# paninski-lab/eks

Hardware: AMD Instinct MI355X
Metric: frames*keypoints smoothed/s + achieved HBM GB/s fraction, singlecam 100k x 256 (higher is better)
Workload: dtype f32

## Files before the change

eks_amd/csrc/eks_diag.hip:

```cpp
#include <hip/hip_runtime.h>

#include <cstdlib>

#include "eks_diag_lane.hpp"
#include "eks_internal.hpp"
#include "eks_win_walk.hpp"

namespace eks {

struct LaneMap {
  int N, T, nc;
  int nt_log2;
  int ntile;
  int reverse;
};

__device__ __forceinline__ bool lane_coords(const LaneMap& L, int& n, int& j) {
  const int wave = blockIdx.x * (blockDim.x >> 6) + (threadIdx.x >> 6);
  const int lane = threadIdx.x & 63;
  const int tile = wave % L.ntile;
  const int cg = wave / L.ntile;
  const int nt = 1 << L.nt_log2;
  n = tile * nt + (lane & (nt - 1));
  j = cg * (64 >> L.nt_log2) + (lane >> L.nt_log2);
// ... 404 lines not shown
}

template <int B, bool UNIT, int VS_ROW>
__device__ __forceinline__ void replay_window_block(const BlockMap& L, const DiagModel& M, const WinWs& Wn,
                                                    const float* __restrict__ y, const float* __restrict__ var,
                                                    float* __restrict__ ms, float* __restrict__ Vs) {
  __shared__ float sh[5][kWinW][64];
  __shared__ float shy[64];
  const int w = __builtin_amdgcn_readfirstlane(threadIdx.x >> 6), lane = threadIdx.x & 63;
  const int tile = L.tile0 + blockIdx.x % L.ntile;
  int wg = blockIdx.x / L.ntile;
  if (L.reverse) wg = Wn.nwg - 1 - wg;
  const int n = tile * 64 + lane;
  constexpr int VW = VS_ROW == 0 ? 1 : VS_ROW;
  const bool slow = n >= L.N || (Wn.slow != nullptr && Wn.slow[n] != 0);
  if (__ballot(!slow) == 0) return;
  const int jh0 = wg * kWinG - kWinH;
  const int j = jh0 + w;
  const bool valid = j >= 0 && j < L.nc;
  const bool live = n < L.N && valid;
  ChainParams<float> p{1.f, 1.f, 0.f};
  const int t0 = valid ? j * B : 0;
  const int len = valid ? min(B, L.T - t0) : 0;
  const bool full = len == B;
  const size_t first = (size_t)t0 * L.N + (size_t)tile * 64;
  const BufferRows rows{rows_rsrc(y + first), rows_rsrc(var + first), (unsigned)lane * 4, (unsigned)L.N * 4};
  float v0[B], v1[B];
  Elem<float> own = elem_identity<float>();
  float y0 = 0.f;
  if (live) {
    p = load_chain_params(M, n);
    if (full) {
      load_rows<B, true>(rows, B, v0, v1);
      y0 = v0[0];
      own = summarize_loaded<B, UNIT, true>(v0, v1, B, p);
    } else {
      load_rows<B, false>(rows, len, v0, v1);
      y0 = v0[0];
      own = summarize_loaded<B, UNIT, false>(v0, v1, len, p);
    }
  }
  sh[0][w][lane] = own.A; sh[1][w][lane] = own.b; sh[2][w][lane] = own.C; sh[3][w][lane] = own.eta;
  sh[4][w][lane] = own.J;
  if (w == 0) shy[lane] = y0;
  __syncthreads();
  const int wo = w - kWinH;
  if (wo < 0 || wo >= kWinG || !live) return;
  auto lds_elem = [&](int q) {
    return Elem<float>{sh[0][q][lane], sh[1][q][lane], sh[2][q][lane], sh[3][q][lane], sh[4][q][lane]};
  };
  const bool cut_front = jh0 <= 0, cut_back = (wg + 1) * kWinG + kWinH >= L.nc;
  Elem<float> hf = lds_elem(0), hb = lds_elem(kWinH + kWinG);
#pragma unroll
  for (int q = 1; q < kWinH; ++q) {
    hf = elem_combine(hf, lds_elem(q));
    hb = elem_combine(hb, lds_elem(kWinH + kWinG + q));
  }
  float m, P;
  load_chain_prior(M, n, m, P);
  if (!cut_front) m = UNIT ? shy[lane] : shy[lane] * rcp(p.c);
  const bool good = !slow && fabsf(m) <= 3e38f && (cut_front || fabsf(hf.A) <= kWinTol) &&
                    (cut_back || fabsf(hb.A) <= kWinTol);
  if (!good && !slow && wo == 0 && Wn.fail != nullptr) {
    Wn.fail[(size_t)wg * L.N + n] = 1;
    atomicOr(&Wn.gate[tile], 1);
  }
  elem_apply(hf, m, P);
  for (int q = 0; q < wo; ++q) elem_apply(lds_elem(kWinH + q), m, P);
  if (full) filter_loaded<B, UNIT, true>(v0, v1, B, p, m, P);
  else filter_loaded<B, UNIT, false>(v0, v1, len, p, m, P);
  float eta = 0.f, J = 0.f;
  elem_back(hb, eta, J);
  for (int q = kWinG - 1; q > wo; --q) elem_back(lds_elem(kWinH + q), eta, J);
  fuse_info(m, P, eta, J);
  if (Wn.nan_bad && !good) m = P = __builtin_nanf("");
  const BufferStore<VS_ROW> st{rows_rsrc(ms + first), rows_rsrc(Vs + first * VW), (unsigned)lane * 4,
                               (unsigned)L.N * 4, n % M.D};
  if (good || Wn.nan_bad) {
    if (full) smooth_rows<B, UNIT, true>(v0, v1, B, p, m, P, st);
    else smooth_rows<B, UNIT, false>(v0, v1, len, p, m, P, st);
  }
}

template <int B, bool UNIT, int VS_ROW>
__device__ __forceinline__ void replay_walk_block(const BlockMap& L, const DiagModel& M, const WinWs& Wn,
                                                  const float* __restrict__ y, const float* __restrict__ var,
                                                  float* __restrict__ ms, float* __restrict__ Vs) {
  __shared__ float sh[5][kWalkRing][64];
  __shared__ float shy[kWalkStand][64];
  const int w = __builtin_amdgcn_readfirstlane(threadIdx.x >> 6), lane = threadIdx.x & 63;
  const int tile = L.tile0 + blockIdx.x % L.ntile;
  const int run_len = Wn.run_len;
  int run = blockIdx.x / L.ntile;
  if (L.reverse) run = (Wn.nwg + run_len - 1) / run_len - 1 - run;
  const int n = tile * 64 + lane;
  constexpr int VW = VS_ROW == 0 ? 1 : VS_ROW;
  const bool slow = n >= L.N || (Wn.slow != nullptr && Wn.slow[n] != 0);
  if (__ballot(!slow) == 0) return;
  ChainParams<float> p{1.f, 1.f, 0.f};
  float m0 = 0.f, P0 = 0.f;
  if (n < L.N) {
    p = load_chain_params(M, n);
    load_chain_prior(M, n, m0, P0);
  }
  const int d = n % M.D;
  float v0[B], v1[B];
  const int g0 = run * run_len, g1 = min(g0 + run_len, Wn.nwg);
  for (int g = g0; g < g1; ++g) {
    const int base = walk_base(g);
    const int off = walk_off(g, w);
    const int j = base + off;
    const bool valid = j >= 0 && j < L.nc;
    const bool live = n < L.N && valid;
    const int t0 = valid ? j * B : 0;
    const int len = valid ? min(B, L.T - t0) : 0;
    const bool full = len == B;
    const size_t first = (size_t)t0 * L.N + (size_t)tile * 64;
    if (walk_loads(off, g == g0)) {
      Elem<float> own = elem_identity<float>();
      float y0 = 0.f;
      if (live) {
        const BufferRows rows{rows_rsrc(y + first), rows_rsrc(var + first), (unsigned)lane * 4, (unsigned)L.N * 4};
        if (full) {
          load_rows<B, true>(rows, B, v0, v1);
          y0 = v0[0];
          own = summarize_loaded<B, UNIT, true>(v0, v1, B, p);
        } else {
          load_rows<B, false>(rows, len, v0, v1);
          y0 = v0[0];
          own = summarize_loaded<B, UNIT, false>(v0, v1, len, p);
        }
      }
      const int slot = walk_elem_slot(j);
      sh[0][slot][lane] = own.A; sh[1][slot][lane] = own.b; sh[2][slot][lane] = own.C; sh[3][slot][lane] = own.eta;
      sh[4][slot][lane] = own.J;
      if (walk_saves_stand(j)) shy[walk_stand_slot(j)][lane] = y0;
    }
    __syncthreads();
    if (!walk_replays(off) || !live) continue;
    const int wo = off - kWinH;
    auto lds_elem = [&](int jj) {
      const int q = walk_elem_slot(jj);
      return Elem<float>{sh[0][q][lane], sh[1][q][lane], sh[2][q][lane], sh[3][q][lane], sh[4][q][lane]};
    };
    const bool cut_front = base <= 0, cut_back = (g + 1) * kWinG + kWinH >= L.nc;
    Elem<float> hf = lds_elem(base), hb = lds_elem(base + kWinH + kWinG);
#pragma unroll
    for (int q = 1; q < kWinH; ++q) {
      hf = elem_combine(hf, lds_elem(base + q));
      hb = elem_combine(hb, lds_elem(base + kWinH + kWinG + q));
    }
    float m = m0, P = P0;
    if (!cut_front) {
      const float ys = shy[walk_stand_slot(base)][lane];
      m = UNIT ? ys : ys * rcp(p.c);
    }
    const bool good = !slow && fabsf(m) <= 3e38f && (cut_front || fabsf(hf.A) <= kWinTol) &&
                      (cut_back || fabsf(hb.A) <= kWinTol);
    if (!good && !slow && wo == 0 && Wn.fail != nullptr) {
      Wn.fail[(size_t)g * L.N + n] = 1;
      atomicOr(&Wn.gate[tile], 1);
    }
    elem_apply(hf, m, P);
    for (int q = 0; q < wo; ++q) elem_apply(lds_elem(base + kWinH + q), m, P);
    if (full) filter_loaded<B, UNIT, true>(v0, v1, B, p, m, P);
    else filter_loaded<B, UNIT, false>(v0, v1, len, p, m, P);
    float eta = 0.f, J = 0.f;
    elem_back(hb, eta, J);
    for (int q = kWinG - 1; q > wo; --q) elem_back(lds_elem(base + kWinH + q), eta, J);
    fuse_info(m, P, eta, J);
    if (Wn.nan_bad && !good) m = P = __builtin_nanf("");
    const BufferStore<VS_ROW> st{rows_rsrc(ms + first), rows_rsrc(Vs + first * VW), (unsigned)lane * 4,
                                 (unsigned)L.N * 4, d};
    if (good || Wn.nan_bad) {
      if (full) smooth_rows<B, UNIT, true>(v0, v1, B, p, m, P, st);
      else smooth_rows<B, UNIT, false>(v0, v1, len, p, m, P, st);
    }
  }
}

constexpr int kFormElems = 0;
constexpr int kFormRecompute = 1;
constexpr int kFormWindow = 2;
constexpr int kFormWalk = 3;

template <int B, bool UNIT, int VS_ROW, int FORM>
__global__ __launch_bounds__(FORM >= kFormWindow ? 64 * kWinW : 64 * kFW) void diag_replay_blk_kernel(
    BlockMap L, DiagModel M, DiagWs W, ScanWs S, WinWs Wn, const float* __restrict__ y, const float* __restrict__ var,
    float* __restrict__ ms, float* __restrict__ Vs) {
  if constexpr (FORM == kFormWalk) {
    replay_walk_block<B, UNIT, VS_ROW>(L, M, Wn, y, var, ms, Vs);
  } else if constexpr (FORM == kFormWindow) {
    replay_window_block<B, UNIT, VS_ROW>(L, M, Wn, y, var, ms, Vs);
  } else if constexpr (FORM == kFormRecompute) {
    replay_recompute_block<B, UNIT, VS_ROW, false>(L, M, S, Wn, y, var, ms, Vs);
  } else {
    const int w = __builtin_amdgcn_readfirstlane(threadIdx.x >> 6), lane = threadIdx.x & 63;
    const int tile = L.tile0 + blockIdx.x % L.ntile;
    int grp = blockIdx.x / L.ntile;
    if (L.reverse) grp = L.ngrp - 1 - grp;
    const int n = tile * 64 + lane, j = grp * kFW + w;
    const int j0 = grp * kFW, j1 = min(j0 + kFW, L.nc);
    constexpr int VW = VS_ROW == 0 ? 1 : VS_ROW;
    if (n >= L.N || j >= L.nc) return;
    const ChainParams<float> p = load_chain_params(M, n);
    const int t0 = j * B;
    const int len = min(B, L.T - t0);
    const bool full = len == B;
    const size_t first = (size_t)t0 * L.N + (size_t)tile * 64;
    const BufferRows rows{rows_rsrc(y + first), rows_rsrc(var + first), (unsigned)lane * 4, (unsigned)L.N * 4};
    float v0[B], v1[B];
    if (full) load_rows<B, true>(rows, B, v0, v1);
    else load_rows<B, false>(rows, len, v0, v1);
    Elem<float> ef[kFW - 1];
#pragma unroll
    for (int q = 0; q < kFW - 1; ++q)
      if (j0 + q < j) ef[q] = load_elem(W, (size_t)(j0 + q) * L.N + n);
    const size_t ob = (size_t)grp * L.N + n;
    float m = S.bm[ob], P = S.bP[ob], eta = S.bEta[ob], J = S.bJ[ob];
#pragma unroll
    for (int q = 0; q < kFW - 1; ++q)
      if (j0 + q < j) elem_apply(ef[q], m, P);
    Elem<float> eb[kFW - 1];
#pragma unroll
    for (int q = 0; q < kFW - 1; ++q)
      if (j + 1 + q < j1) eb[q] = load_elem(W, (size_t)(j + 1 + q) * L.N + n);
    if (full) filter_loaded<B, UNIT, true>(v0, v1, B, p, m, P);
    else filter_loaded<B, UNIT, false>(v0, v1, len, p, m, P);
#pragma unroll
    for (int q = kFW - 2; q >= 0; --q)
      if (j + 1 + q < j1) elem_back(eb[q], eta, J);
    fuse_info(m, P, eta, J);
    const BufferStore<VS_ROW> st{rows_rsrc(ms + first), rows_rsrc(Vs + first * VW), (unsigned)lane * 4,
                                 (unsigned)L.N * 4, n % M.D};
    if (full) smooth_rows<B, UNIT, true>(v0, v1, B, p, m, P, st);
    else smooth_rows<B, UNIT, false>(v0, v1, len, p, m, P, st);
  }
}

template <int B, bool UNIT, int VS_ROW>
__global__ __launch_bounds__(64 * kFW) void diag_replay_exact_kernel(BlockMap L, DiagModel M, ScanWs S, WinWs Wn,
                                                                    const float* __restrict__ y,
                                                                    const float* __restrict__ var,
                                                                    float* __restrict__ ms,
                                                                    float* __restrict__ Vs) {
  replay_recompute_block<B, UNIT, VS_ROW, true>(L, M, S, Wn, y, var, ms, Vs);
}

__global__ __launch_bounds__(64 * kProbeWin) void diag_window_probe_kernel(int N, int T, DiagModel M, WinWs Wn,
                                                                          const float* __restrict__ var,
                                                                          int classify) {
  __shared__ int bad[kProbeWin][64];
  const int w = __builtin_amdgcn_readfirstlane(threadIdx.x >> 6), lane = threadIdx.x & 63;
  const int tile = blockIdx.x, n = tile * 64 + lane;
  for (int i = threadIdx.x; i < Wn.nwg * 64; i += 64 * kProbeWin) {
    const int c = tile * 64 + (i & 63);
    if (c < N) Wn.fail[(size_t)(i >> 6) * N + c] = 0;
  }
  int s = 0;
  if (classify && n < N) {
    const ChainParams<float> p = load_chain_params(M, n);
    const int t0 = (int)((long long)w * (T - kProbeLen) / (kProbeWin - 1));
    const float* v = var + (size_t)t0 * N + n;
    float r[kProbeLen];
#pragma unroll
    for (int i = 0; i < kProbeLen; ++i) r[i] = v[(size_t)i * N];
    float A = 1.f, C = 0.f;
#pragma unroll
    for (int i = 0; i < kProbeLen; ++i) {
      const float ri = clip_var(r[i]);
      const float rg = ri * rcp(ri + C * p.c * p.c);
      A = p.times_a(A * rg);
      C = p.times_a2(C * rg) + p.q_s;
    }
// ... 78 lines not shown
#pragma unroll
    for (int i = 0; i < PER; ++i)
      if (b0 + i < q1) {
        const size_t o = (size_t)(b0 + i) * N + n;
        S.bm[o] = m;
        S.bP[o] = P;
        elem_apply(e[i], m, P);
      }
  }
  for (int b1 = q1; b1 > q0; b1 -= PER) {
    const int lo = max(q0, b1 - PER);
    if (!held) {
#pragma unroll
      for (int i = 0; i < PER; ++i)
        if (lo + i < b1) e[i] = agg(lo + i);
    }
#pragma unroll
    for (int i = PER - 1; i >= 0; --i)
      if (lo + i < b1) {
        const size_t o = (size_t)(lo + i) * N + n;
        S.bEta[o] = eta;
        S.bJ[o] = J;
        elem_back(e[i], eta, J);
      }
  }
}

#ifndef EKS_DIAG_CHUNK
#define EKS_DIAG_CHUNK 32
#endif
constexpr int kChunk = EKS_DIAG_CHUNK;

static inline size_t plane_bytes(int nc, int N) { return align_up((size_t)nc * N * sizeof(float), 256); }

static inline size_t win_slow_bytes(int N) { return align_up((size_t)N, 256); }
static inline size_t win_fail_bytes(int nc, int N) { return align_up((size_t)((nc + kWinG - 1) / kWinG) * N, 256); }
static inline size_t win_bytes(int nc, int N) {
  return win_slow_bytes(N) + win_fail_bytes(nc, N) + align_up((size_t)((N + 63) / 64) * sizeof(int), 256);
}

size_t diag_smooth_workspace_bytes(int T, int N) {
  const int nc = (T + kChunk - 1) / kChunk;
  const int nblk = (nc + kFW - 1) / kFW;
  return 9 * plane_bytes(nc, N) + 9 * plane_bytes(nblk, N) + win_bytes(nc, N);
}

static LaneMap make_lane_map(int T, int N, int B) {
  LaneMap L;
  L.N = N;
  L.T = T;
  L.nc = (T + B - 1) / B;
  int nt_log2 = 0;
  while ((1 << nt_log2) < N && nt_log2 < 6) ++nt_log2;
  L.nt_log2 = nt_log2;
  L.ntile = (N + (1 << nt_log2) - 1) >> nt_log2;
  L.reverse = 0;
  return L;
}

template <bool UNIT>
static void launch_replay(int vs_row, dim3 grid, hipStream_t st, const LaneMap& L, const DiagModel& M,
                          const DiagWs& W, const float* y, const float* var, float* ms, float* Vs) {
#define EKS_REPLAY(R)                                                                             \
  case R:                                                                                         \
    hipLaunchKernelGGL((diag_replay_kernel<kChunk, UNIT, R>), grid, dim3(256), 0, st, L, M, W, y, \
                       var, ms, Vs);                                                              \
    break;
  switch (vs_row) {
    EKS_REPLAY(0)
    EKS_REPLAY(1)
    EKS_REPLAY(2)
    EKS_REPLAY(3)
    EKS_REPLAY(4)
    EKS_REPLAY(5)
    EKS_REPLAY(6)
    EKS_REPLAY(7)
    EKS_REPLAY(8)
  }
#undef EKS_REPLAY
}

constexpr int kWalkDefault = 1;
constexpr int kWalkMinRun = 2;

static int device_cu_count() {
  static const int n = [] {
    int dev = 0, c = 0;
    if (hipGetDevice(&dev) != hipSuccess ||
        hipDeviceGetAttribute(&c, hipDeviceAttributeMultiprocessorCount, dev) != hipSuccess || c <= 0)
      c = 256;
    return c;
  }();
  return n;
}

static int walk_run(int ntile, int nwg) {
  if (knob_int(KNOB_SMOOTH_WINDOW_WALK, kWalkDefault) == 0) return 0;
  if (knob_set(KNOB_SMOOTH_WINDOW_RUN)) return min(max(knob_int(KNOB_SMOOTH_WINDOW_RUN, 1), 1), nwg);
  thread_local int c_ntile = 0, c_nwg = 0, c_run = 0;
  if (ntile != c_ntile || nwg != c_nwg) {
    c_run = walk_run_length(ntile, nwg, device_cu_count());
    c_ntile = ntile;
    c_nwg = nwg;
  }
  return c_run >= kWalkMinRun ? c_run : 0;
}

int diag_smooth(const eks_dims_t& d, const float* y, const float* var, const DiagModel& M,
                float* ms, float* Vs, void* ws, size_t ws_bytes, hipStream_t st) {
  const int T = d.n_frames, D = d.state_dim, N = d.n_keypoints * D;
  const bool vs_diag = d.flags & EKS_FLAG_VS_DIAG;
  if (!vs_diag && D > 8) return EKS_ERR_UNSUPPORTED;
  if (ws_bytes < diag_smooth_workspace_bytes(T, N)) return EKS_ERR_WORKSPACE;
  const LaneMap Lf = make_lane_map(T, N, kChunk);
  const LaneMap& L = Lf;
  const size_t pb = plane_bytes(L.nc, N);
  char* base = static_cast<char*>(ws);
  DiagWs W;
  float** planes[9] = {&W.eA, &W.eb, &W.eC, &W.eEta, &W.eJ, &W.pm, &W.pP, &W.sEta, &W.sJ};
  for (int i = 0; i < 9; ++i) *planes[i] = reinterpret_cast<float*>(base + i * pb);
  const int ngrp_f = (L.nc + kFW - 1) / kFW;
  const bool in_range = (size_t)kChunk * N * (vs_diag ? 1 : D) * sizeof(float) < ((size_t)1 << 31);
  const bool fused = L.nt_log2 == 6 && in_range &&
                     (knob_set(KNOB_SMOOTH_UNFUSED) ? knob_int(KNOB_SMOOTH_UNFUSED, 0) == 0 : ngrp_f <= 1024);
  ScanWs S;
  S.nblk = fused ? (L.nc + kFW - 1) / kFW : (L.nc + kScanCB - 1) / kScanCB;
  const size_t sb = plane_bytes(S.nblk, N);
  float** splanes[9] = {&S.gA, &S.gb, &S.gC, &S.gEta, &S.gJ, &S.bm, &S.bP, &S.bEta, &S.bJ};
  for (int i = 0; i < 9; ++i) *splanes[i] = reinterpret_cast<float*>(base + 9 * pb + i * sb);
  const int vs_row = vs_diag ? 0 : D;
  const bool unit = d.flags & EKS_FLAG_UNIT_AC;
  const int k1_reverse = knob_int(KNOB_SUMMARIZE_REVERSE, 0) == 1 ? 1 : 0;
  const int k3_reverse = knob_set(KNOB_REPLAY_FORWARD) ? (knob_int(KNOB_REPLAY_FORWARD, 0) == 1 ? 0 : 1) : !k1_reverse;
  const int win_mode = knob_int(KNOB_SMOOTH_WINDOW, kWinDefault);
  const int win_min_t = max(kProbeLen, knob_int(KNOB_SMOOTH_WINDOW_MIN_T, kWinMinT));
  const bool windowed = fused && win_mode != 0 && T >= win_min_t;
  WinWs Wn{nullptr, nullptr, nullptr, (L.nc + kWinG - 1) / kWinG, 0, 0};
  if (windowed) {
    char* wb = base + 9 * pb + 9 * sb;
    if (win_mode == 2) {
      Wn.nan_bad = 1;
    } else {
      Wn.slow = reinterpret_cast<unsigned char*>(wb);
      Wn.fail = reinterpret_cast<unsigned char*>(wb + win_slow_bytes(N));
      Wn.gate = reinterpret_cast<int*>(wb + win_slow_bytes(N) + win_fail_bytes(L.nc, N));
    }
  }
  const int* gate = windowed ? Wn.gate : nullptr;
  if (fused) {
    const bool rc_all = knob_set(KNOB_REPLAY_RECOMPUTE) ? knob_int(KNOB_REPLAY_RECOMPUTE, 0) == 1
                                                        : 5 * pb >= ((size_t)16 << 20);
    const int tp = L.ntile;
    for (int tile0 = 0; tile0 < L.ntile; tile0 += tp) {
    const int ntl = min(tp, L.ntile - tile0);
    const int n0 = tile0 * 64, Np = min(N - n0, ntl * 64);
    BlockMap Bm{N, T, L.nc, ntl, S.nblk, k1_reverse, tile0};
    const dim3 bgrid((unsigned)((long)Bm.ntile * Bm.ngrp)), bblock(64 * kFW);
    const bool rc = rc_all || windowed;
#define EKS_K1_BLK(UN)                                                                                  \
  do {                                                                                                  \
    if (rc)                                                                                             \
      hipLaunchKernelGGL((diag_summarize_blk_kernel<kChunk, UN, true>), bgrid, bblock, 0, st, Bm, M, W, \
                         S, y, var, gate);                                                              \
    else                                                                                                \
      hipLaunchKernelGGL((diag_summarize_blk_kernel<kChunk, UN, false>), bgrid, bblock, 0, st, Bm, M,   \
                         W, S, y, var, gate);                                                           \
  } while (0)
#define EKS_K3_BLK(UN, R)                                                                               \
  do {                                                                                                  \
    if (windowed)                                                                                       \
      hipLaunchKernelGGL((diag_replay_exact_kernel<kChunk, UN, R>), bgrid, bblock, 0, st, Bm, M, S, Wn, \
                         y, var, ms, Vs);                                                               \
    else if (rc)                                                                                        \
      hipLaunchKernelGGL((diag_replay_blk_kernel<kChunk, UN, R, kFormRecompute>), bgrid, bblock, 0, st, \
                         Bm, M, W, S, Wn, y, var, ms, Vs);                                              \
    else                                                                                                \
      hipLaunchKernelGGL((diag_replay_blk_kernel<kChunk, UN, R, kFormElems>), bgrid, bblock, 0, st, Bm, \
                         M, W, S, Wn, y, var, ms, Vs);                                                  \
  } while (0)
#define EKS_K3_WIN(UN, R)                                                                               \
  hipLaunchKernelGGL((diag_replay_blk_kernel<kChunk, UN, R, kFormWindow>), wgrid, dim3(64 * kWinW), 0,  \
                     st, Bw, M, W, S, Wn, y, var, ms, Vs)
#define EKS_K3_WALK(UN, R)                                                                             \
  hipLaunchKernelGGL((diag_replay_blk_kernel<kChunk, UN, R, kFormWalk>), wgrid, dim3(64 * kWinW), 0,    \
                     st, Bw, M, W, S, Ww, y, var, ms, Vs)
#define EKS_REPLAY_WIN(R)                                                                              \
  case R:                                                                                              \
    if (run_len > 0) {                                                                                 \
      if (unit)                                                                                        \
        EKS_K3_WALK(true, R);                                                                          \
      else                                                                                             \
        EKS_K3_WALK(false, R);                                                                         \
    } else if (unit)                                                                                   \
      EKS_K3_WIN(true, R);                                                                             \
    else                                                                                               \
      EKS_K3_WIN(false, R);                                                                            \
    break;
    if (windowed) {
      if (win_mode != 2) {
        ProfScope ps("diag_window_probe", st);
        hipLaunchKernelGGL(diag_window_probe_kernel, dim3(ntl), dim3(64 * kProbeWin), 0, st, N, T, M, Wn, var,
                           knob_int(KNOB_SMOOTH_WINDOW_PROBE, 1) != 0 ? 1 : 0);
      }
      {
        ProfScope ps("diag_replay", st);
        BlockMap Bw = Bm;
        Bw.reverse = k3_reverse;
        const int run_len = walk_run(Bw.ntile, Wn.nwg);
        WinWs Ww = Wn;
        Ww.run_len = run_len;
        const dim3 wgrid((unsigned)((long)Bw.ntile * (run_len > 0 ? (Wn.nwg + run_len - 1) / run_len : Wn.nwg)));
        switch (vs_row) {
          EKS_REPLAY_WIN(0)
          EKS_REPLAY_WIN(1)
          EKS_REPLAY_WIN(2)
          EKS_REPLAY_WIN(3)
          EKS_REPLAY_WIN(4)
          EKS_REPLAY_WIN(5)
          EKS_REPLAY_WIN(6)
          EKS_REPLAY_WIN(7)
          EKS_REPLAY_WIN(8)
        }
      }
      if (win_mode == 2) continue;
    }
    {
      ProfScope ps("diag_summarize", st);
      if (unit)
        EKS_K1_BLK(true);
      else
        EKS_K1_BLK(false);
    }
    {
      ProfScope ps("diag_scan", st);
      const bool ch4 = knob_set(KNOB_SCAN_CH) ? knob_int(KNOB_SCAN_CH, 4) == 4 : Np < 2048;
      const bool per8 = (S.nblk + 63) / 64 <= 8;
      const int Ne = n0 + Np;
      if (ch4) {
        if (per8)
          hipLaunchKernelGGL((diag_scan_groups_kernel<8, 4>), dim3((Np + 3) / 4), dim3(256), 0, st, N, n0, Ne, M, S, gate);
        else
          hipLaunchKernelGGL((diag_scan_groups_kernel<16, 4>), dim3((Np + 3) / 4), dim3(256), 0, st, N, n0, Ne, M, S, gate);
      } else {
        if (per8)
          hipLaunchKernelGGL((diag_scan_groups_kernel<8, 16>), dim3((Np + 15) / 16), dim3(1024), 0, st, N, n0, Ne, M, S, gate);
        else
          hipLaunchKernelGGL((diag_scan_groups_kernel<16, 16>), dim3((Np + 15) / 16), dim3(1024), 0, st, N, n0, Ne, M, S, gate);
      }
    }
    ProfScope ps(windowed ? "diag_replay_exact" : "diag_replay", st);
    Bm.reverse = k3_reverse;
#define EKS_REPLAY_BLK(R)                                                                              \
  case R:                                                                                              \
    if (unit)                                                                                          \
      EKS_K3_BLK(true, R);                                                                             \
    else                                                                                               \
      EKS_K3_BLK(false, R);                                                                            \
    break;
    switch (vs_row) {
      EKS_REPLAY_BLK(0)
      EKS_REPLAY_BLK(1)
      EKS_REPLAY_BLK(2)
      EKS_REPLAY_BLK(3)
      EKS_REPLAY_BLK(4)
      EKS_REPLAY_BLK(5)
      EKS_REPLAY_BLK(6)
      EKS_REPLAY_BLK(7)
      EKS_REPLAY_BLK(8)
    }
    }
#undef EKS_REPLAY_BLK
#undef EKS_REPLAY_WIN
#undef EKS_K3_WIN
#undef EKS_K3_WALK
#undef EKS_K3_BLK
#undef EKS_K1_BLK
    return hip_status(hipGetLastError());
  }

  const int cpw = 64 >> L.nt_log2;
  const long waves = (long)L.ntile * ((L.nc + cpw - 1) / cpw);
  const dim3 grid((unsigned)((waves + 3) / 4));
  {
    ProfScope ps("diag_summarize", st);
    LaneMap L = Lf;
    L.reverse = k1_reverse;
    if (unit)
      hipLaunchKernelGGL((diag_summarize_kernel<kChunk, true>), grid, dim3(256), 0, st, L, M, W, y, var);
    else
      hipLaunchKernelGGL((diag_summarize_kernel<kChunk, false>), grid, dim3(256), 0, st, L, M, W, y, var);
  }
  {
    ProfScope ps("diag_scan", st);
    const dim3 sgrid((N + kScanCH - 1) / kScanCH, S.nblk), sblock(kScanCH * kScanCB);
    hipLaunchKernelGGL(diag_scan_reduce_kernel, sgrid, sblock, 0, st, N, L.nc, W, S);
    hipLaunchKernelGGL(diag_scan_blocks_kernel, dim3((N + 3) / 4), dim3(256), 0, st, N, M, S);
    hipLaunchKernelGGL(diag_scan_local_kernel, sgrid, sblock, 0, st, N, L.nc, W, S);
  }
  {
    ProfScope ps("diag_replay", st);
    LaneMap L = Lf;
    L.reverse = k3_reverse;
    if (unit)
      launch_replay<true>(vs_row, grid, st, L, M, W, y, var, ms, Vs);
    else
      launch_replay<false>(vs_row, grid, st, L, M, W, y, var, ms, Vs);
  }
  return hip_status(hipGetLastError());
}

}

EKS_DEFINE_TOUCH(diag)
```

eks_amd/csrc/eks_internal.hpp:

```cpp
#pragma once
#include <hip/hip_runtime.h>

#include <cstddef>
#include <cstdint>

#include "../../include/eks_hip.h"

namespace eks {

struct DiagModel;

static inline size_t align_up(size_t x, size_t a) { return (x + a - 1) / a * a; }
static inline int hip_status(hipError_t e) { return e == hipSuccess ? EKS_OK : EKS_ERR_HIP_BASE - (int)e; }

__device__ __forceinline__ int xcd_contiguous_block(int b, int nb) {
  const int x = b & 7, i = b >> 3, q = nb >> 3, r = nb & 7;
  return x * q + (x < r ? x : r) + i;
}

enum Knob {
  KNOB_SMOOTH_UNFUSED, KNOB_SUMMARIZE_REVERSE, KNOB_REPLAY_FORWARD, KNOB_REPLAY_RECOMPUTE, KNOB_SCAN_CH,
  KNOB_DENSE_CHUNK, KNOB_NLL_NCL, KNOB_NLL_CHUNK, KNOB_NLL_CHUNK0, KNOB_NLL_WPB,
  KNOB_DENSE_LEGACY, KNOB_NLL_GRAD_UNFUSED, KNOB_NLL_GRAD_CHUNK,
  KNOB_DENSE_TREE_SCAN, KNOB_DENSE_DUAL_GRAD, KNOB_NLL_LEGACY, KNOB_MED_ROWS, KNOB_DW_CHUNK, KNOB_ADAM_PER_ITERATION, KNOB_MED_FINISH_THREADS, KNOB_MED_BRACKET_THREADS, KNOB_NLL_NOLAG, KNOB_NLL_GRAD_TREE, KNOB_ADAM_STREAM, KNOB_ADAM_LAG_RHO_PPM, KNOB_ADAM_LAG_HEAD,
  KNOB_SMOOTH_WINDOW, KNOB_SMOOTH_WINDOW_MIN_T, KNOB_SMOOTH_WINDOW_PROBE,
  KNOB_SMOOTH_WINDOW_WALK, KNOB_SMOOTH_WINDOW_RUN, KNOB_COUNT
};
bool knob_set(Knob k);
int knob_int(Knob k, int dflt);

#define EKS_DEFINE_TOUCH(unit)                                                                              \
  namespace eks {                                                                                           \
  __global__ void touch_##unit##_kernel() {}                                                                \
  void touch_##unit() {                                                                                     \
    hipFuncAttributes a;                                                                                    \
    (void)hipFuncGetAttributes(&a, reinterpret_cast<const void*>(touch_##unit##_kernel));                   \
  }                                                                                                         \
  }
void touch_misc();
void touch_diag();
void touch_diag_nll();
void touch_dense();
void touch_dense_wave();
void touch_dense_wide();
void touch_loss();
void touch_loss_ar1();
void touch_multicam();
void touch_lag_adam();

class ProfScope {
 public:
  ProfScope(const char* name, hipStream_t st);
  ~ProfScope();

 private:
  const char* name_;
  hipStream_t st_;
  bool live_;
  hipEvent_t a_, b_;
};

size_t diag_smooth_workspace_bytes(int T, int N);
int diag_smooth(const eks_dims_t& d, const float* y, const float* var, const DiagModel& M,
                float* ms, float* Vs, void* ws, size_t ws_bytes, hipStream_t st);
size_t diag_nll_workspace_bytes(int T, int N, int n_cand);
struct AdamFuse;
int diag_nll(const eks_dims_t& d, const float* y, const double* rconst, const DiagModel& M,
             const double* s_cand, int n_cand, int per_keypoint, double* nll, double* dnll,
             void* ws, size_t ws_bytes, hipStream_t st, const AdamFuse* fuse = nullptr, double* s_out = nullptr,
             int32_t* idx_out = nullptr);
bool diag_nll_grad_tree(int T, int K, int D);
bool diag_nll_adam_persist_ok(int T, int K, int D, int n_blocks);
int diag_nll_adam_persist(const eks_dims_t& d, const float* y, const double* rconst, const DiagModel& M, int n_iters,
                          double* nll, double* dnll, const AdamFuse& F, int32_t* n_active, hipStream_t st);
bool diag_lag_adam_ok(int T, int K, int D, int n_blocks);
size_t diag_lag_adam_workspace_bytes(int T, int N);
int diag_lag_sums(const eks_dims_t& d, const float* y, const double* A, const AdamFuse* F, void* ws, size_t ws_bytes,
                  hipStream_t st);
int diag_lag_adam(const eks_dims_t& d, const float* y, const double* rconst, const DiagModel& M, int n_iters, double* nll,
                  double* dnll, const AdamFuse& F, void* ws, size_t ws_bytes, hipStream_t st);
size_t adam_extra_bytes(int N);
int32_t* nll_ws_tickets(void* ws, int T, int N, int n_cand);
int adam_prepare(int n_blocks, int K, const int32_t* offs, const int32_t* members, int32_t* kp_block,
                 int32_t* counter_a, int32_t* counter_b, hipStream_t st);

bool diag_chain_covers(int T, int N);

size_t diag_sample_workspace_bytes(int T, int N, int n_draws);
int diag_sample(const eks_dims_t& d, const float* y, const float* var, const DiagModel& M, int n_draws, uint64_t seed,
                int first_keypoint, int first_draw, const float* noise, float* ms, float* draws, void* ws,
                size_t ws_bytes, hipStream_t st);
int diag_sample_noise(int T, int N, int D, int n_draws, uint64_t seed, int first_keypoint, int first_draw, float* noise,
                      hipStream_t st);
struct DenseModel;
size_t dense_sample_workspace_bytes(int T, int K, int D, int O, int n_draws);
int dense_sample(const eks_dims_t& d, const float* y, const float* var, const DenseModel& M, int n_draws, uint64_t seed,
                 int first_keypoint, int first_draw, const float* noise, float* ms, float* draws, void* ws,
                 size_t ws_bytes, hipStream_t st);
int dense_sample_noise(int T, int K, int W, int n_draws, uint64_t seed, int first_keypoint, int first_draw, float* noise,
                       hipStream_t st);

struct DenseModel {
  const double *m0, *S0, *A, *C, *Q, *s;
};
size_t diag_increments_workspace_bytes(int T, int N);
int diag_increments(const eks_dims_t& d, const float* y, const float* var, const DiagModel& M, float* ms, float* Vs,
                    float* lag1, float* dmean, float* dV, void* ws, size_t ws_bytes, hipStream_t st);
size_t dense_increments_workspace_bytes(int T, int K, int D, int O);
int dense_increments(const eks_dims_t& d, const float* y, const float* var, const DenseModel& M, float* ms, float* Vs,
// ... 141 lines not shown
```

eks_amd/csrc/eks_profile.hip:

```cpp
#include <hip/hip_runtime.h>

#include <cstdlib>
#include <cstring>
#include <mutex>
#include <vector>

#include "eks_internal.hpp"

namespace eks {

namespace {
struct KnobTable {
  bool set[KNOB_COUNT];
  int val[KNOB_COUNT];
  KnobTable() { load(); }
  int load() {
    static const char* const names[KNOB_COUNT] = {
        "EKS_SMOOTH_UNFUSED", "EKS_SUMMARIZE_REVERSE", "EKS_REPLAY_FORWARD", "EKS_REPLAY_RECOMPUTE", "EKS_SCAN_CH",
        "EKS_DENSE_CHUNK", "EKS_NLL_NCL", "EKS_NLL_CHUNK", "EKS_NLL_CHUNK0", "EKS_NLL_WPB",
        "EKS_DENSE_LEGACY", "EKS_NLL_GRAD_UNFUSED",
        "EKS_NLL_GRAD_CHUNK", "EKS_DENSE_TREE_SCAN", "EKS_DENSE_DUAL_GRAD", "EKS_NLL_LEGACY", "EKS_MED_ROWS", "EKS_DW_CHUNK", "EKS_ADAM_PER_ITERATION", "EKS_MED_FINISH_THREADS", "EKS_MED_BRACKET_THREADS", "EKS_NLL_NOLAG", "EKS_NLL_GRAD_TREE", "EKS_ADAM_STREAM", "EKS_ADAM_LAG_RHO_PPM", "EKS_ADAM_LAG_HEAD",
        "EKS_SMOOTH_WINDOW", "EKS_SMOOTH_WINDOW_MIN_T", "EKS_SMOOTH_WINDOW_PROBE",
        "EKS_SMOOTH_WINDOW_WALK", "EKS_SMOOTH_WINDOW_RUN"};
    int n = 0;
    for (int i = 0; i < KNOB_COUNT; ++i) {
      const char* v = getenv(names[i]);
      set[i] = v != nullptr;
      val[i] = v ? atoi(v) : 0;
      n += set[i];
    }
    return n;
  }
};
KnobTable& knob_table() {
  static KnobTable t;
  return t;
}
}

bool knob_set(Knob k) { return knob_table().set[k]; }
int knob_int(Knob k, int dflt) { return knob_table().set[k] ? knob_table().val[k] : dflt; }

struct ProfEntry {
  const char* name;
  hipEvent_t a, b;
};
static int g_prof_level = 0;
static std::vector<ProfEntry> g_prof;
static std::vector<hipEvent_t> g_pool;
static std::mutex g_prof_mu;

static hipEvent_t take_event() {
  std::lock_guard<std::mutex> lk(g_prof_mu);
  if (!g_pool.empty()) {
    hipEvent_t e = g_pool.back();
    g_pool.pop_back();
    return e;
  }
  hipEvent_t e;
  hipEventCreate(&e);
  return e;
}

static bool scope_live(const char* name) {
  if (g_prof_level == 1) return true;
  if (g_prof_level != 2) return false;
  const size_t n = strlen(name);
  return (n >= 7 && strcmp(name + n - 7, "_replay") == 0) || strcmp(name, "diag_nll_summarize") == 0;
}

ProfScope::ProfScope(const char* name, hipStream_t st) : name_(name), st_(st), live_(scope_live(name)) {
  if (!live_) return;
  a_ = take_event();
  b_ = take_event();
  hipEventRecord(a_, st_);
}
ProfScope::~ProfScope() {
  if (!live_) return;
  hipEventRecord(b_, st_);
  std::lock_guard<std::mutex> lk(g_prof_mu);
  g_prof.push_back({name_, a_, b_});
}

}

extern "C" {

int eks_knobs_reload(void) { return eks::knob_table().load(); }

int eks_profile_enable(int on) {
  eks::g_prof_level = on < 0 ? 0 : on > 2 ? 1 : on;
  return EKS_OK;
}

int eks_profile_drain(char* names, size_t names_bytes, float* ms, int32_t max_n) {
  std::lock_guard<std::mutex> lk(eks::g_prof_mu);
  int n = 0;
  size_t off = 0;
  for (auto& e : eks::g_prof) {
    hipEventSynchronize(e.b);
    float t = 0.f;
    hipEventElapsedTime(&t, e.a, e.b);
    eks::g_pool.push_back(e.a);
    eks::g_pool.push_back(e.b);
    const size_t len = strlen(e.name) + 1;
    if (n < max_n && names && ms && off + len <= names_bytes) {
// ... 11 lines not shown
```

eks_amd/csrc/eks_win_walk.hpp:

```cpp
#pragma once

namespace eks {

#ifndef EKS_WIN_G
#define EKS_WIN_G 8
#endif
constexpr int kWinG = EKS_WIN_G;
constexpr int kWinH = 2;
constexpr int kWinW = kWinG + 2 * kWinH;
static_assert(kWinG >= 2 * kWinH, "the carried chunks of a step and the chunks whose elements the next step's front "
                                  "halo needs are different own chunks");

constexpr int kWalkRing = 2 * kWinW;
constexpr int kWalkStand = 3;

constexpr int walk_base(int g) { return g * kWinG - kWinH; }
constexpr int walk_wave(int j) { return (j + kWinW) % kWinW; }
constexpr int walk_off(int g, int w) { return (w + kWinW - walk_wave(walk_base(g))) % kWinW; }
constexpr int walk_chunk(int g, int w) { return walk_base(g) + walk_off(g, w); }
constexpr bool walk_loads(int off, bool first_step) { return first_step || off >= 2 * kWinH; }
constexpr bool walk_replays(int off) { return off >= kWinH && off < kWinH + kWinG; }
constexpr bool walk_keeps(int off) { return off >= kWinH + kWinG; }
constexpr int walk_elem_slot(int j) { return (j + kWalkRing) % kWalkRing; }
constexpr bool walk_saves_stand(int j) { return (j + kWinH) % kWinG == 0; }
constexpr int walk_stand_slot(int j) { return ((j + kWinH) / kWinG) % kWalkStand; }

constexpr int kWalkRunEnd = 1;
constexpr int walk_run_length(int ntile, int nwg, int ncu) {
  long best = -1;
  int br = 1;
  for (int r = 1; r <= nwg; ++r) {
    const long blocks = (long)ntile * ((nwg + r - 1) / r);
    const long cost = ((blocks + ncu - 1) / ncu) * (r + kWalkRunEnd);
    if (best < 0 || cost < best) {
      best = cost;
      br = r;
    }
  }
  return br;
}

}
```

Before: 60.11 billion.

## Prefetch next walk step's input rows into LDS via buffer-load-to-LDS

Adds a staged variant of the walk replay kernel, enabled by default. Waves issue asynchronous buffer_load_lds prefetches of the y/var rows for the chunk they will load on the next step, so the global-memory latency overlaps the current step's replay. The next step then reads the rows from LDS instead of global memory. A wide variant uses 16-byte loads that cover four rows per instruction when pointers are aligned. This costs extra LDS (kWinG slots of 2*B*64 floats), which may reduce occupancy, and adds vmcnt(0) waits. Optional timestamp instrumentation is included behind a macro.

New measurement: 59.94 billion. About the same (-0.3%).

```diff
diff --git a/eks_amd/csrc/eks_diag.hip b/eks_amd/csrc/eks_diag.hip
--- a/eks_amd/csrc/eks_diag.hip
+++ b/eks_amd/csrc/eks_diag.hip
@@ -510,12 +510,103 @@
   }
 }
 
-template <int B, bool UNIT, int VS_ROW>
+#ifndef EKS_STAGE_AUX
+#define EKS_STAGE_AUX kAuxNt
+#endif
+#ifndef EKS_STAGE_WIDE
+#define EKS_STAGE_WIDE 1
+#endif
+template <int B, bool FULL>
+__device__ __forceinline__ void stage_rows(const BufferRows& rows, int len, float (*dst)[B][64]) {
+  typedef __attribute__((address_space(3))) void lds_void;
+#pragma unroll
+  for (int i = 0; i < B; ++i) {
+    if (FULL || i < len) {
+      __builtin_amdgcn_raw_ptr_buffer_load_lds(rows.ry, (lds_void*)&dst[0][i][0], 4, rows.voff,
+                                               (unsigned)i * rows.row_bytes, 0, EKS_STAGE_AUX);
+      __builtin_amdgcn_raw_ptr_buffer_load_lds(rows.rv, (lds_void*)&dst[1][i][0], 4, rows.voff,
+                                               (unsigned)i * rows.row_bytes, 0, EKS_STAGE_AUX);
+    }
+  }
+}
+
+template <int B, bool FULL>
+__device__ __forceinline__ void stage_rows_wide(const BufferRows& rows, int len, int lane, float (*dst)[B][64]) {
+  typedef __attribute__((address_space(3))) void lds_void;
+  static_assert(B % 4 == 0, "four rows per instruction");
+  const int r = lane >> 4;
+  const unsigned voff = (unsigned)r * rows.row_bytes + (unsigned)(lane & 15) * 16;
+#pragma unroll
+  for (int i = 0; i < B; i += 4) {
+    if (FULL || i < len) {
+      if (FULL || i + r < len) {
+        __builtin_amdgcn_raw_ptr_buffer_load_lds(rows.ry, (lds_void*)&dst[0][i][0], 16, voff,
+                                                 (unsigned)i * rows.row_bytes, 0, EKS_STAGE_AUX);
+        __builtin_amdgcn_raw_ptr_buffer_load_lds(rows.rv, (lds_void*)&dst[1][i][0], 16, voff,
+                                                 (unsigned)i * rows.row_bytes, 0, EKS_STAGE_AUX);
+      }
+    }
+  }
+}
+
+template <int B, bool FULL>
+__device__ __forceinline__ void staged_rows(const float (*src)[B][64], int lane, int len, float (&v0)[B],
+                                            float (&v1)[B]) {
+#pragma unroll
+  for (int i = 0; i < B; ++i) {
+    if (FULL || i < len) {
+      v0[i] = src[0][i][lane];
+      v1[i] = src[1][i][lane];
+    }
+  }
+}
+
+#ifdef EKS_WALK_STAMPS
+constexpr int kWalkStampBlocks = 256, kWalkStampSteps = 16;
+__device__ unsigned long long g_walk_stamps[kWalkStampBlocks][kWalkStampSteps][kWinW][10];
+#define WALK_STAMP_NOW(i)                            \
+  do {                                               \
+    __builtin_amdgcn_sched_barrier(0);               \
+    stamp_[i] = __builtin_amdgcn_s_memrealtime();    \
+    __builtin_amdgcn_sched_barrier(0);               \
+  } while (0)
+#define WALK_STAMP_TOP()                             \
+  unsigned long long stamp_[8] = {};                 \
+  WALK_STAMP_NOW(0)
+#define WALK_STAMP(i) WALK_STAMP_NOW(i)
+#define WALK_STAMP_ARRIVED()                         \
+  do {                                               \
+    asm volatile("s_waitcnt vmcnt(0)" ::: "memory"); \
+    WALK_STAMP_NOW(2);                               \
+  } while (0)
+#define WALK_STAMP_AFTER(i, x)                       \
+  do {                                               \
+    asm volatile("" : "+v"(x));                      \
+    WALK_STAMP_NOW(i);                               \
+  } while (0)
+#define WALK_STAMP_FLUSH(off, step)                                                              \
+  do {                                                                                           \
+    if (lane == 0 && blockIdx.x < kWalkStampBlocks && (step) < kWalkStampSteps) {                \
+      unsigned long long* st_ = g_walk_stamps[blockIdx.x][step][w];                              \
+      for (int i_ = 0; i_ < 8; ++i_) st_[i_] = stamp_[i_];                                       \
+      st_[8] = (unsigned long long)(off) + 1;                                                    \
+    }                                                                                            \
+  } while (0)
+#else
+#define WALK_STAMP_TOP() do { } while (0)
+#define WALK_STAMP(i) do { } while (0)
+#define WALK_STAMP_ARRIVED() do { } while (0)
+#define WALK_STAMP_AFTER(i, x) do { } while (0)
+#define WALK_STAMP_FLUSH(off, step) do { } while (0)
+#endif
+
+template <int B, bool UNIT, int VS_ROW, bool STAGE>
 __device__ __forceinline__ void replay_walk_block(const BlockMap& L, const DiagModel& M, const WinWs& Wn,
                                                   const float* __restrict__ y, const float* __restrict__ var,
                                                   float* __restrict__ ms, float* __restrict__ Vs) {
   __shared__ float sh[5][kWalkRing][64];
   __shared__ float shy[kWalkStand][64];
+  __shared__ float stage[kStageSlots][2][B][64];
   const int w = __builtin_amdgcn_readfirstlane(threadIdx.x >> 6), lane = threadIdx.x & 63;
   const int tile = L.tile0 + blockIdx.x % L.ntile;
   const int run_len = Wn.run_len;
@@ -534,6 +625,8 @@
   const int d = n % M.D;
   float v0[B], v1[B];
   const int g0 = run * run_len, g1 = min(g0 + run_len, Wn.nwg);
+  const bool wide = STAGE && UNIT && EKS_STAGE_WIDE &&
+                    ((reinterpret_cast<uintptr_t>(y) | reinterpret_cast<uintptr_t>(var)) & 15) == 0 && L.N % 4 == 0;
   for (int g = g0; g < g1; ++g) {
     const int base = walk_base(g);
     const int off = walk_off(g, w);
@@ -544,28 +637,64 @@
     const int len = valid ? min(B, L.T - t0) : 0;
     const bool full = len == B;
     const size_t first = (size_t)t0 * L.N + (size_t)tile * 64;
+    WALK_STAMP_TOP();
     if (walk_loads(off, g == g0)) {
       Elem<float> own = elem_identity<float>();
       float y0 = 0.f;
       if (live) {
-        const BufferRows rows{rows_rsrc(y + first), rows_rsrc(var + first), (unsigned)lane * 4, (unsigned)L.N * 4};
-        if (full) {
-          load_rows<B, true>(rows, B, v0, v1);
-          y0 = v0[0];
-          own = summarize_loaded<B, UNIT, true>(v0, v1, B, p);
-        } else {
-          load_rows<B, false>(rows, len, v0, v1);
-          y0 = v0[0];
-          own = summarize_loaded<B, UNIT, false>(v0, v1, len, p);
+        bool staged = false;
+        if constexpr (STAGE) {
+          if (stage_consumes(off, g == g0)) {
+            const float(*rows)[B][64] = stage[stage_read_slot(off)];
+            staged = true;
+            WALK_STAMP(1);
+            asm volatile("s_waitcnt vmcnt(0)" ::: "memory");
+            WALK_STAMP(2);
+            if (full) staged_rows<B, true>(rows, lane, B, v0, v1);
+            else staged_rows<B, false>(rows, lane, len, v0, v1);
+          }
         }
+        if (!staged) {
+          const BufferRows rows{rows_rsrc(y + first), rows_rsrc(var + first), (unsigned)lane * 4, (unsigned)L.N * 4};
+          if (full) load_rows<B, true>(rows, B, v0, v1);
+          else load_rows<B, false>(rows, len, v0, v1);
+          WALK_STAMP(1);
+          WALK_STAMP_ARRIVED();
+        }
+        y0 = v0[0];
+        if (full) own = summarize_loaded<B, UNIT, true>(v0, v1, B, p);
+        else own = summarize_loaded<B, UNIT, false>(v0, v1, len, p);
       }
       const int slot = walk_elem_slot(j);
       sh[0][slot][lane] = own.A; sh[1][slot][lane] = own.b; sh[2][slot][lane] = own.C; sh[3][slot][lane] = own.eta;
       sh[4][slot][lane] = own.J;
       if (walk_saves_stand(j)) shy[walk_stand_slot(j)][lane] = y0;
+      WALK_STAMP(3);
     }
     __syncthreads();
-    if (!walk_replays(off) || !live) continue;
+    WALK_STAMP(4);
+    if constexpr (STAGE) {
+      const int jn = j + kWinW;
+      if (stage_prefetches(off, jn, L.nc, g + 1 < g1)) {
+        const int tn = jn * B, lenn = min(B, L.T - tn);
+        const size_t firstn = (size_t)tn * L.N + (size_t)tile * 64;
+        const BufferRows rows{rows_rsrc(y + firstn), rows_rsrc(var + firstn), (unsigned)lane * 4, (unsigned)L.N * 4};
+        if (wide) {
+          if (tile * 64 + 4 * (lane & 15) < L.N) {
+            if (lenn == B) stage_rows_wide<B, true>(rows, B, lane, stage[stage_fill_slot(off)]);
+            else stage_rows_wide<B, false>(rows, lenn, lane, stage[stage_fill_slot(off)]);
+          }
+        } else if (n < L.N) {
+          if (lenn == B) stage_rows<B, true>(rows, B, stage[stage_fill_slot(off)]);
+          else stage_rows<B, false>(rows, lenn, stage[stage_fill_slot(off)]);
+        }
+      }
+      WALK_STAMP(5);
+    }
+    if (!walk_replays(off) || !live) {
+      WALK_STAMP_FLUSH(off, g - g0);
+      continue;
+    }
     const int wo = off - kWinH;
     auto lds_elem = [&](int jj) {
       const int q = walk_elem_slot(jj);
@@ -593,6 +722,7 @@
     for (int q = 0; q < wo; ++q) elem_apply(lds_elem(base + kWinH + q), m, P);
     if (full) filter_loaded<B, UNIT, true>(v0, v1, B, p, m, P);
     else filter_loaded<B, UNIT, false>(v0, v1, len, p, m, P);
+    WALK_STAMP_AFTER(6, m);
     float eta = 0.f, J = 0.f;
     elem_back(hb, eta, J);
     for (int q = kWinG - 1; q > wo; --q) elem_back(lds_elem(base + kWinH + q), eta, J);
@@ -604,6 +734,8 @@
       if (full) smooth_rows<B, UNIT, true>(v0, v1, B, p, m, P, st);
       else smooth_rows<B, UNIT, false>(v0, v1, len, p, m, P, st);
     }
+    WALK_STAMP(7);
+    WALK_STAMP_FLUSH(off, g - g0);
   }
 }
 
@@ -611,13 +743,16 @@
 constexpr int kFormRecompute = 1;
 constexpr int kFormWindow = 2;
 constexpr int kFormWalk = 3;
+constexpr int kFormWalkStage = 4;
 
 template <int B, bool UNIT, int VS_ROW, int FORM>
 __global__ __launch_bounds__(FORM >= kFormWindow ? 64 * kWinW : 64 * kFW) void diag_replay_blk_kernel(
     BlockMap L, DiagModel M, DiagWs W, ScanWs S, WinWs Wn, const float* __restrict__ y, const float* __restrict__ var,
     float* __restrict__ ms, float* __restrict__ Vs) {
-  if constexpr (FORM == kFormWalk) {
-    replay_walk_block<B, UNIT, VS_ROW>(L, M, Wn, y, var, ms, Vs);
+  if constexpr (FORM == kFormWalkStage) {
+    replay_walk_block<B, UNIT, VS_ROW, true>(L, M, Wn, y, var, ms, Vs);
+  } else if constexpr (FORM == kFormWalk) {
+    replay_walk_block<B, UNIT, VS_ROW, false>(L, M, Wn, y, var, ms, Vs);
   } else if constexpr (FORM == kFormWindow) {
     replay_window_block<B, UNIT, VS_ROW>(L, M, Wn, y, var, ms, Vs);
   } else if constexpr (FORM == kFormRecompute) {
@@ -862,6 +997,7 @@
 
 constexpr int kWalkDefault = 1;
 constexpr int kWalkMinRun = 2;
+constexpr int kStageDefault = 1;
 
 static int device_cu_count() {
   static const int n = [] {
@@ -964,9 +1100,17 @@
 #define EKS_K3_WALK(UN, R)                                                                             \
   hipLaunchKernelGGL((diag_replay_blk_kernel<kChunk, UN, R, kFormWalk>), wgrid, dim3(64 * kWinW), 0,    \
                      st, Bw, M, W, S, Ww, y, var, ms, Vs)
+#define EKS_K3_STAGE(UN, R)                                                                            \
+  hipLaunchKernelGGL((diag_replay_blk_kernel<kChunk, UN, R, kFormWalkStage>), wgrid, dim3(64 * kWinW),  \
+                     0, st, Bw, M, W, S, Ww, y, var, ms, Vs)
 #define EKS_REPLAY_WIN(R)                                                                              \
   case R:                                                                                              \
-    if (run_len > 0) {                                                                                 \
+    if (run_len > 0 && staged) {                                                                       \
+      if (unit)                                                                                        \
+        EKS_K3_STAGE(true, R);                                                                         \
+      else                                                                                             \
+        EKS_K3_STAGE(false, R);                                                                        \
+    } else if (run_len > 0) {                                                                          \
       if (unit)                                                                                        \
         EKS_K3_WALK(true, R);                                                                          \
       else                                                                                             \
@@ -987,6 +1131,7 @@
         BlockMap Bw = Bm;
         Bw.reverse = k3_reverse;
         const int run_len = walk_run(Bw.ntile, Wn.nwg);
+        const bool staged = knob_int(KNOB_SMOOTH_WINDOW_STAGE, kStageDefault) != 0;
         WinWs Ww = Wn;
         Ww.run_len = run_len;
         const dim3 wgrid((unsigned)((long)Bw.ntile * (run_len > 0 ? (Wn.nwg + run_len - 1) / run_len : Wn.nwg)));
@@ -1053,6 +1198,7 @@
 #undef EKS_REPLAY_WIN
 #undef EKS_K3_WIN
 #undef EKS_K3_WALK
+#undef EKS_K3_STAGE
 #undef EKS_K3_BLK
 #undef EKS_K1_BLK
     return hip_status(hipGetLastError());
@@ -1091,4 +1237,16 @@
 
 }
 
+#ifdef EKS_WALK_STAMPS
+extern "C" int eks_debug_walk_stamps(unsigned long long* out) {
+  hipError_t e = hipMemcpyFromSymbol(out, HIP_SYMBOL(eks::g_walk_stamps), sizeof(eks::g_walk_stamps));
+  if (e == hipSuccess) {
+    void* p = nullptr;
+    e = hipGetSymbolAddress(&p, HIP_SYMBOL(eks::g_walk_stamps));
+    if (e == hipSuccess) e = hipMemset(p, 0, sizeof(eks::g_walk_stamps));
+  }
+  return (int)e;
+}
+#endif
+
 EKS_DEFINE_TOUCH(diag)
diff --git a/eks_amd/csrc/eks_internal.hpp b/eks_amd/csrc/eks_internal.hpp
--- a/eks_amd/csrc/eks_internal.hpp
+++ b/eks_amd/csrc/eks_internal.hpp
@@ -24,7 +24,7 @@
   KNOB_DENSE_LEGACY, KNOB_NLL_GRAD_UNFUSED, KNOB_NLL_GRAD_CHUNK,
   KNOB_DENSE_TREE_SCAN, KNOB_DENSE_DUAL_GRAD, KNOB_NLL_LEGACY, KNOB_MED_ROWS, KNOB_DW_CHUNK, KNOB_ADAM_PER_ITERATION, KNOB_MED_FINISH_THREADS, KNOB_MED_BRACKET_THREADS, KNOB_NLL_NOLAG, KNOB_NLL_GRAD_TREE, KNOB_ADAM_STREAM, KNOB_ADAM_LAG_RHO_PPM, KNOB_ADAM_LAG_HEAD,
   KNOB_SMOOTH_WINDOW, KNOB_SMOOTH_WINDOW_MIN_T, KNOB_SMOOTH_WINDOW_PROBE,
-  KNOB_SMOOTH_WINDOW_WALK, KNOB_SMOOTH_WINDOW_RUN, KNOB_COUNT
+  KNOB_SMOOTH_WINDOW_WALK, KNOB_SMOOTH_WINDOW_RUN, KNOB_SMOOTH_WINDOW_STAGE, KNOB_COUNT
 };
 bool knob_set(Knob k);
 int knob_int(Knob k, int dflt);
diff --git a/eks_amd/csrc/eks_profile.hip b/eks_amd/csrc/eks_profile.hip
--- a/eks_amd/csrc/eks_profile.hip
+++ b/eks_amd/csrc/eks_profile.hip
@@ -21,7 +21,7 @@
         "EKS_DENSE_LEGACY", "EKS_NLL_GRAD_UNFUSED",
         "EKS_NLL_GRAD_CHUNK", "EKS_DENSE_TREE_SCAN", "EKS_DENSE_DUAL_GRAD", "EKS_NLL_LEGACY", "EKS_MED_ROWS", "EKS_DW_CHUNK", "EKS_ADAM_PER_ITERATION", "EKS_MED_FINISH_THREADS", "EKS_MED_BRACKET_THREADS", "EKS_NLL_NOLAG", "EKS_NLL_GRAD_TREE", "EKS_ADAM_STREAM", "EKS_ADAM_LAG_RHO_PPM", "EKS_ADAM_LAG_HEAD",
         "EKS_SMOOTH_WINDOW", "EKS_SMOOTH_WINDOW_MIN_T", "EKS_SMOOTH_WINDOW_PROBE",
-        "EKS_SMOOTH_WINDOW_WALK", "EKS_SMOOTH_WINDOW_RUN"};
+        "EKS_SMOOTH_WINDOW_WALK", "EKS_SMOOTH_WINDOW_RUN", "EKS_SMOOTH_WINDOW_STAGE"};
     int n = 0;
     for (int i = 0; i < KNOB_COUNT; ++i) {
       const char* v = getenv(names[i]);
diff --git a/eks_amd/csrc/eks_win_walk.hpp b/eks_amd/csrc/eks_win_walk.hpp
--- a/eks_amd/csrc/eks_win_walk.hpp
+++ b/eks_amd/csrc/eks_win_walk.hpp
@@ -25,6 +25,14 @@
 constexpr bool walk_saves_stand(int j) { return (j + kWinH) % kWinG == 0; }
 constexpr int walk_stand_slot(int j) { return ((j + kWinH) / kWinG) % kWalkStand; }
 
+constexpr int kStageSlots = kWinG;
+constexpr bool stage_prefetches(int off, int j_next, int nc, bool next_in_run) {
+  return off < kWinG && next_in_run && j_next >= 0 && j_next < nc;
+}
+constexpr int stage_fill_slot(int off) { return off; }
+constexpr bool stage_consumes(int off, bool first_step) { return !first_step && off >= 2 * kWinH; }
+constexpr int stage_read_slot(int off) { return off - 2 * kWinH; }
+
 constexpr int kWalkRunEnd = 1;
 constexpr int walk_run_length(int ntile, int nwg, int ncu) {
   long best = -1;
```
